# cxjyxxme/deep-online-video-stabilization

Measured on NVIDIA B200. Metric: warp_fwd_bwd_mpix_per_s, higher is better.
Workload: dtype f32

## Files before the change

### deep-online-video-stabilization_b200/csrc/mgw_warp_tma.cu

```cuda
#include "mgw_tile.cuh"

#ifdef MGW_PROBE
__device__ unsigned long long g_probe[16];
extern "C" __attribute__((visibility("default"))) int mgw_debug_probe(unsigned long long* out, int reset)
{
    cudaDeviceSynchronize();
    cudaMemcpyFromSymbol(out, g_probe, sizeof(g_probe));
    if (reset) { unsigned long long z[16] = {}; cudaMemcpyToSymbol(g_probe, z, sizeof(z)); }
    return 0;
}
#define PROBE(i) do { if (threadIdx.x == MGW_PROBE_TID) { const long long t_ = clock64(); atomicAdd(&g_probe[i], (unsigned long long)(t_ - tprev)); tprev = t_; } } while (0)
#else
#define PROBE(i) do {} while (0)
#endif
#ifndef MGW_PROBE_TID
#define MGW_PROBE_TID 32
#endif

namespace mgw {

constexpr int kMaxWarps = 16;

template <int C, int TW, int K, int NT>
struct Geo {
    static constexpr int kGroups = NT / TW;
    static constexpr int TH = kGroups * K;
    static constexpr int kXalign = (C % 4 == 0) ? 1 : ((C % 2 == 0) ? 2 : 4);
    static constexpr int kWantF = (((TW * 13 + 9) / 10 + 4 + (kXalign - 1)) * C + 31) / 32 * 32;
    static constexpr int kRowF = kWantF < 256 ? kWantF : 256;
    static constexpr int SBW = kRowF / C;
    static constexpr int SBH = (TH * 13 + 9) / 10 + 4;
    static constexpr int kBoxF = SBH * kRowF;
    static constexpr int kOutF = (TH * TW * C + 31) / 32 * 32;
    static_assert(SBW >= TW + 4, "source box too narrow for this tile width / channel count");
};

struct TileInfo {
    int bx0, by0;
    int interior;
    float wmax[kMaxWarps];
};

struct Tile {
    int n, r0, c0, vr0, vc0, cell, part;
};

__device__ __forceinline__ Tile this_tile(const TileCfg& cfg)
{
    Tile t;
    const int ty = blockIdx.y, tx = blockIdx.x;
    t.n = blockIdx.z;
    t.r0 = cfg.rows.start[ty]; t.vr0 = cfg.rows.vstart[ty];
    t.c0 = cfg.cols.start[tx]; t.vc0 = cfg.cols.vstart[tx];
    t.cell = (t.n * cfg.gh + cfg.rows.cell[ty]) * cfg.gw + cfg.cols.cell[tx];
    t.part = cfg.rows.part[ty] * cfg.parts_x + cfg.cols.part[tx];
    return t;
}

template <int C, int TW, int K, int NT>
__device__ __forceinline__ void source_box(const TileCfg& cfg, const Tile& tl, const float (&Hc)[9], float stepx, float stepy,
                                           int& bx0, int& by0, int& interior, int* complete = nullptr)
{
    using G = Geo<C, TW, K, NT>;
    const int k4 = threadIdx.x & 3;
    const int rr = tl.r0 + ((k4 & 2) ? G::TH - 1 : 0), cc = tl.c0 + ((k4 & 1) ? TW - 1 : 0);
    const Proj q = project(Hc, lin_at(cc, stepx), lin_at(rr, stepy));
    const float x = (q.xn + 1.0f) * (float)cfg.W * 0.5f, y = (q.yn + 1.0f) * (float)cfg.H * 0.5f;
    bool ok = (fabsf(x) < 1.0e8f) && (fabsf(y) < 1.0e8f);
    int sgn = (q.zs > 0.0f) ? 1 : -1;
    float xmin = x, xmax = x, ymin = y, ymax = y;
#pragma unroll
    for (int o = 1; o < 4; o <<= 1) {
        xmin = fminf(xmin, __shfl_xor_sync(0xffffffffu, xmin, o));
        xmax = fmaxf(xmax, __shfl_xor_sync(0xffffffffu, xmax, o));
        ymin = fminf(ymin, __shfl_xor_sync(0xffffffffu, ymin, o));
        ymax = fmaxf(ymax, __shfl_xor_sync(0xffffffffu, ymax, o));
        sgn += __shfl_xor_sync(0xffffffffu, sgn, o);
        ok = ok && (__shfl_xor_sync(0xffffffffu, (int)ok, o) != 0);
    }
    ok = ok && (sgn == 4 || sgn == -4);
    bx0 = 0; by0 = 0; interior = 0;
    if (complete) *complete = 0;
    if (ok) {
        const int ux0 = (int)floorf(xmin) - 1, ux1 = (int)floorf(xmax) + 2;
        const int uy0 = (int)floorf(ymin) - 1, uy1 = (int)floorf(ymax) + 2;
        const int ix0 = clipi(ux0, 0, cfg.W - 1), ix1 = clipi(ux1, 0, cfg.W - 1);
        const int iy0 = clipi(uy0, 0, cfg.H - 1), iy1 = clipi(uy1, 0, cfg.H - 1);
        const int needw = ix1 - ix0 + 1, needh = iy1 - iy0 + 1;
        bx0 = needw <= G::SBW ? ix0 : ix0 + (needw - G::SBW) / 2;
        by0 = needh <= G::SBH ? iy0 : iy0 + (needh - G::SBH) / 2;
        bx0 -= bx0 % G::kXalign;
        interior = (ux0 >= 0 && ux1 <= cfg.W - 1 && uy0 >= 0 && uy1 <= cfg.H - 1 &&
                    ux1 - bx0 < G::SBW && uy1 - by0 < G::SBH) ? 1 : 0;
        if (complete) *complete = (ix0 >= bx0 && ix1 - bx0 < G::SBW && iy0 >= by0 && iy1 - by0 < G::SBH) ? 1 : 0;
    }
}

struct FastTaps { int x0, y0; float ax, bx, ay, by; };
__device__ __forceinline__ FastTaps make_taps_interior(float xn, float yn, int IH, int IW)
{
    const float x = __fmul_rn(__fmul_rn(__fadd_rn(xn, 1.0f), (float)IW), 0.5f);
    const float y = __fmul_rn(__fmul_rn(__fadd_rn(yn, 1.0f), (float)IH), 0.5f);
    const float fx = floorf(x), fy = floorf(y);
    FastTaps t;
    t.x0 = __float2int_rz(fx); t.y0 = __float2int_rz(fy);
    t.ax = __fsub_rn(__fadd_rn(fx, 1.0f), x); t.bx = __fsub_rn(x, fx);
    t.ay = __fsub_rn(__fadd_rn(fy, 1.0f), y); t.by = __fsub_rn(y, fy);
    return t;
}

__device__ __forceinline__ float blend4(float ax, float bx, float ay, float by, float Ia, float Ib, float Ic, float Id)
{
    const float wa = __fmul_rn(ax, ay), wb = __fmul_rn(ax, by), wc = __fmul_rn(bx, ay), wd = __fmul_rn(bx, by);
    float s = __fmul_rn(wa, Ia);
    s = __fadd_rn(s, __fmul_rn(wb, Ib));
    s = __fadd_rn(s, __fmul_rn(wc, Ic));
    s = __fadd_rn(s, __fmul_rn(wd, Id));
    return s;
}

#ifndef MGW_FWD_MINB
#define MGW_FWD_MINB (NT == 256 ? (LOSS ? 3 : 4) : 2)
#endif
template <int C, int TW, int K, int NT, bool LOSS>
__global__ void __launch_bounds__(NT, MGW_FWD_MINB)
warp_fwd_tma_kernel(const __grid_constant__ CUtensorMap mapU, const __grid_constant__ CUtensorMap mapOut,
                    const float* __restrict__ U, const float* __restrict__ Hs, const __grid_constant__ TileCfg cfg,
                    float* __restrict__ out, float* __restrict__ img, float* __restrict__ black,
                    const float* __restrict__ y_tgt, float* __restrict__ sums)
{
    using G = Geo<C, TW, K, NT>;
    extern __shared__ __align__(1024) unsigned char smem_raw[];
    float* s_src = reinterpret_cast<float*>(smem_raw);
    float* s_out = s_src + G::kBoxF;
    uint64_t* bar = reinterpret_cast<uint64_t*>(s_out + G::kOutF);
    TileInfo* ti = reinterpret_cast<TileInfo*>(bar + 2);

    const int tid = threadIdx.x;
    if (tid == 0) {
        tma::mbar_init(bar, 1);
        tma::fence_barrier_init();
    }
    const Tile tl = this_tile(cfg);
    float Hc[9];
#pragma unroll
    for (int k = 0; k < 9; ++k) Hc[k] = __ldg(Hs + (size_t)tl.cell * 9 + k);
    const float stepx = cfg.stepx, stepy = cfg.stepy;
    __syncthreads();
    if (tid < 32 && out) {
        int bx0, by0, interior;
        source_box<C, TW, K, NT>(cfg, tl, Hc, stepx, stepy, bx0, by0, interior);
        if (tid == 0) {
            ti->bx0 = bx0; ti->by0 = by0; ti->interior = interior;
            tma::mbar_expect_tx(bar, (uint32_t)(G::kBoxF * sizeof(float)));
            tma::load_3d(s_src, &mapU, bar, bx0 * C, by0, tl.n);
        }
    }

    const int tx = tid % TW, g = tid / TW;
    const float xt = lin_at(tl.c0 + tx, stepx);
    const float hx0 = __fmul_rn(Hc[0], xt), hx3 = __fmul_rn(Hc[3], xt), hx6 = __fmul_rn(Hc[6], xt);
    float xn[K], yn[K];
    float yv[LOSS ? K : 1][C], nbv[LOSS ? K : 1];
    {
        size_t p = ((size_t)tl.n * cfg.H + tl.r0 + g * K) * cfg.W + tl.c0 + tx;
#pragma unroll
        for (int k = 0; k < K; ++k, p += cfg.W) {
            if (LOSS) {
#pragma unroll
                for (int ch = 0; ch < C; ++ch) yv[k][ch] = __ldg(y_tgt + p * C + ch);
            }
            const float yt = lin_at(tl.r0 + g * K + k, stepy);
            const float xs = __fadd_rn(__fmaf_rn(Hc[1], yt, hx0), Hc[2]);
            const float ys = __fadd_rn(__fmaf_rn(Hc[4], yt, hx3), Hc[5]);
            float zs = __fadd_rn(__fmaf_rn(Hc[7], yt, hx6), Hc[8]);
            zs = __fadd_rn(zs, (zs >= 0.0f) ? 1e-8f : -1e-8f);
            div2_rn(xs, ys, zs, xn[k], yn[k]);
            const float bk = black_of(xn[k], yn[k]);
            if (img) reinterpret_cast<float2*>(img)[p] = make_float2(xn[k], yn[k]);
            if (black) black[p] = bk;
            if (LOSS) nbv[k] = (tl.r0 + g * K + k >= tl.vr0 && tl.c0 + tx >= tl.vc0) ? 1.0f - bk : -1.0f;
        }
    }
    if (!out) return;
    float se = 0.0f, sm = 0.0f;
    tma::mbar_wait(bar, 0);
    const int bx0 = ti->bx0, by0 = ti->by0;
    if (ti->interior) {
#pragma unroll
        for (int k = 0; k < K; ++k) {
            const FastTaps t = make_taps_interior(xn[k], yn[k], cfg.H, cfg.W);
            const float* pa = s_src + ((t.y0 - by0) * G::kRowF + (t.x0 - bx0) * C);
            float* o = s_out + ((g * K + k) * TW + tx) * C;
#pragma unroll
            for (int ch = 0; ch < C; ++ch) {
                const float v = blend4(t.ax, t.bx, t.ay, t.by, pa[ch], pa[G::kRowF + ch], pa[C + ch], pa[G::kRowF + C + ch]);
                o[ch] = v;
                if (LOSS && nbv[k] >= 0.0f) { const float e = (v - yv[k][ch]) * nbv[k]; se = fmaf(e, e, se); }
            }
            if (LOSS && nbv[k] >= 0.0f) sm += nbv[k];
        }
    } else {
        const float* Un = U + (size_t)tl.n * cfg.H * cfg.W * C;
#pragma unroll
        for (int k = 0; k < K; ++k) {
            const Taps t = make_taps(xn[k], yn[k], cfg.H, cfg.W);
            const int sx0 = t.x0 - bx0, sx1 = t.x1 - bx0, sy0 = t.y0 - by0, sy1 = t.y1 - by0;
            float* o = s_out + ((g * K + k) * TW + tx) * C;
            if (sx0 >= 0 && sx1 < G::SBW && sy0 >= 0 && sy1 < G::SBH) {
                const float* pa = s_src + sy0 * G::kRowF + sx0 * C;
                const float* pb = s_src + sy1 * G::kRowF + sx0 * C;
                const float* pc = s_src + sy0 * G::kRowF + sx1 * C;
                const float* pd = s_src + sy1 * G::kRowF + sx1 * C;
#pragma unroll
                for (int ch = 0; ch < C; ++ch) o[ch] = blend(t, pa[ch], pb[ch], pc[ch], pd[ch]);
            } else {
                const float* pa = Un + ((size_t)t.y0 * cfg.W + t.x0) * C;
                const float* pb = Un + ((size_t)t.y1 * cfg.W + t.x0) * C;
                const float* pc = Un + ((size_t)t.y0 * cfg.W + t.x1) * C;
                const float* pd = Un + ((size_t)t.y1 * cfg.W + t.x1) * C;
#pragma unroll
                for (int ch = 0; ch < C; ++ch) o[ch] = blend(t, __ldg(pa + ch), __ldg(pb + ch), __ldg(pc + ch), __ldg(pd + ch));
            }
            if (LOSS && nbv[k] >= 0.0f) {
#pragma unroll
                for (int ch = 0; ch < C; ++ch) { const float e = (o[ch] - yv[k][ch]) * nbv[k]; se = fmaf(e, e, se); }
                sm += nbv[k];
            }
        }
    }
    if (LOSS) {
        se = warp_sum(se); sm = warp_sum(sm);
        float* s_loss = reinterpret_cast<float*>(ti + 1);
        if ((tid & 31) == 0) { s_loss[(tid >> 5) * 2] = se; s_loss[(tid >> 5) * 2 + 1] = sm; }
    }
    tma::fence_proxy_async();
    __syncthreads();
    if (tid == 0) {
        tma::store_3d(&mapOut, s_out, tl.c0 * C, tl.r0, tl.n);
        tma::commit_group();
        if (LOSS) {
            const float* s_loss = reinterpret_cast<const float*>(ti + 1);
            float a = 0.0f, b = 0.0f;
#pragma unroll
            for (int w = 0; w < NT / 32; ++w) { a += s_loss[2 * w]; b += s_loss[2 * w + 1]; }
            atomicAdd(sums + 2 * tl.n, a);
            atomicAdd(sums + 2 * tl.n + 1, b);
        }
        tma::wait_group_read0();
    }
}

constexpr float kMagic = 12582912.0f;
constexpr int kMagicBits = 0x4B400000;
__device__ __forceinline__ int fixed_of(float w, float gs) { return __float_as_int(__fmaf_rn(w, gs, kMagic)) - kMagicBits; }
__device__ __forceinline__ float float_of_fixed(int v) { return (float)v; }
constexpr int bit_width(int v) { return v > 0 ? 1 + bit_width(v >> 1) : 0; }

__device__ __forceinline__ void accumulate_dh(float (&dh)[8], float gxn, float gyn, float xn, float yn, float zs, float xt, float yt)
{
    const float rz = __frcp_rn(zs);
    const float dxs = gxn * rz, dys = gyn * rz;
    const float dzs = -(gxn * xn + gyn * yn) * rz;
    dh[0] = fmaf(dxs, xt, dh[0]); dh[1] = fmaf(dxs, yt, dh[1]); dh[2] += dxs;
    dh[3] = fmaf(dys, xt, dh[3]); dh[4] = fmaf(dys, yt, dh[4]); dh[5] += dys;
    dh[6] = fmaf(dzs, xt, dh[6]); dh[7] = fmaf(dzs, yt, dh[7]);
}

__device__ __forceinline__ void accumulate_dh_r(float (&dh)[8], float gxn, float gyn, float xn, float yn, float rz, float xt, float yt)
{
    const float dxs = gxn * rz, dys = gyn * rz;
    const float dzs = -(gxn * xn + gyn * yn) * rz;
    dh[0] = fmaf(dxs, xt, dh[0]); dh[1] = fmaf(dxs, yt, dh[1]); dh[2] += dxs;
    dh[3] = fmaf(dys, xt, dh[3]); dh[4] = fmaf(dys, yt, dh[4]); dh[5] += dys;
    dh[6] = fmaf(dzs, xt, dh[6]); dh[7] = fmaf(dzs, yt, dh[7]);
}

struct LossBwd {
    const float* out;
    const float* y;
    const float* black;
    const float* sums;
    float kscale;
    const float* kscale_dev;
};

#ifndef MGW_BWD_MINB
#define MGW_BWD_MINB (NT == 256 ? (K <= 3 ? 4 : 3) : 2)
#endif
#ifndef MGW_BWD_NODU_MINB
#define MGW_BWD_NODU_MINB (NT == 256 ? 4 : 2)
#endif
template <int C, int TW, int K, int NT, bool LOSS, bool DU>
__global__ void __launch_bounds__(NT, DU ? MGW_BWD_MINB : MGW_BWD_NODU_MINB)
warp_bwd_tma_kernel(const __grid_constant__ CUtensorMap mapU, const __grid_constant__ CUtensorMap mapG,
                    const __grid_constant__ CUtensorMap mapGI, const float* __restrict__ U, const float* __restrict__ Hs, const float* __restrict__ d_out,
                    const float* __restrict__ d_img, const __grid_constant__ TileCfg cfg, float* __restrict__ dU,
                    float* __restrict__ parts, const LossBwd loss)
{
    using G = Geo<C, TW, K, NT>;
    extern __shared__ __align__(1024) unsigned char smem_raw[];
    float* s_src = reinterpret_cast<float*>(smem_raw);
    float* s_red = s_src + G::kBoxF;
    uint64_t* bar = reinterpret_cast<uint64_t*>(s_red + 128);
    TileInfo* ti = reinterpret_cast<TileInfo*>(bar + 2);
    int* s_acc = reinterpret_cast<int*>(s_red + 256);

    constexpr bool STAGE = DU && !LOSS && (G::kBoxF >= G::TH * TW * (C + 2));
    constexpr int kStageOut = G::TH * TW * C;
    const int tid = threadIdx.x, lane = tid & 31, warp = tid >> 5;
#ifdef MGW_PROBE
    long long tprev = clock64();
    if (tid == MGW_PROBE_TID) atomicAdd(&g_probe[15], 1ull);
#endif
    if (tid == 0) {
        tma::mbar_init(bar, 1);
        if (STAGE) tma::mbar_init(bar + 1, 1);
        tma::fence_barrier_init();
    }
    griddep_launch_dependents();
    PROBE(11);
    const Tile tl = this_tile(cfg);
    PROBE(12);
    if (STAGE && tid == 0) {
        float* sg = reinterpret_cast<float*>(s_acc);
        tma::mbar_expect_tx(bar + 1, (uint32_t)((kStageOut + (d_img ? G::TH * TW * 2 : 0)) * sizeof(float)));
        tma::load_3d(sg, &mapG, bar + 1, tl.c0 * C, tl.r0, tl.n);
        if (d_img) tma::load_3d(sg + kStageOut, &mapGI, bar + 1, tl.c0 * 2, tl.r0, tl.n);
    }
    float Hc[9];
#pragma unroll
    for (int k = 0; k < 9; ++k) Hc[k] = __ldg(Hs + (size_t)tl.cell * 9 + k);
    const float stepx = cfg.stepx, stepy = cfg.stepy;
    const int tx = tid % TW, g = tid / TW;
    const int col = tl.c0 + tx;

    if (tid < 32) {
        int bx0, by0, interior, complete;
        source_box<C, TW, K, NT>(cfg, tl, Hc, stepx, stepy, bx0, by0, interior, &complete);
        if (tid == 0) {
            ti->bx0 = bx0; ti->by0 = by0; ti->interior = complete;
            tma::mbar_expect_tx(bar, (uint32_t)(G::kBoxF * sizeof(float)));
            tma::load_3d(s_src, &mapU, bar, bx0 * C, by0, tl.n);
        }
    }
    PROBE(13);
    float gout[K][C], gimg[K][2];
    if (STAGE) {
        __syncthreads();
        tma::mbar_wait(bar + 1, 0);
        const float* sg = reinterpret_cast<const float*>(s_acc) + (g * K * TW + tx) * C;
        const float2* si = reinterpret_cast<const float2*>(reinterpret_cast<const float*>(s_acc) + kStageOut) + g * K * TW + tx;
#pragma unroll
        for (int k = 0; k < K; ++k) {
#pragma unroll
            for (int ch = 0; ch < C; ++ch) gout[k][ch] = sg[k * TW * C + ch];
            if (d_img) {
                const float2 di = si[k * TW];
                gimg[k][0] = di.x; gimg[k][1] = di.y;
            } else {
                gimg[k][0] = 0.0f; gimg[k][1] = 0.0f;
            }
        }
    } else {
        size_t p = ((size_t)tl.n * cfg.H + tl.r0 + g * K) * cfg.W + col;
        const float kn = LOSS ? (loss.kscale_dev ? loss.kscale * __ldg(loss.kscale_dev) : loss.kscale) / (__ldg(loss.sums + 2 * tl.n + 1) + 1e-8f) : 0.0f;
#pragma unroll
        for (int k = 0; k < K; ++k, p += cfg.W) {
            if (LOSS) {
                const float nb = 1.0f - __ldg(loss.black + p);
                const float kk = kn * nb * nb;
#pragma unroll
                for (int ch = 0; ch < C; ++ch) {
                    gout[k][ch] = kk * (__ldg(loss.out + p * C + ch) - __ldg(loss.y + p * C + ch));
                    if (d_out) gout[k][ch] += __ldg(d_out + p * C + ch);
                }
            } else {
#pragma unroll
                for (int ch = 0; ch < C; ++ch) gout[k][ch] = __ldg(d_out + p * C + ch);
            }
            if (d_img) {
                const float2 di = __ldg(reinterpret_cast<const float2*>(d_img) + p);
                gimg[k][0] = di.x; gimg[k][1] = di.y;
            } else {
                gimg[k][0] = 0.0f; gimg[k][1] = 0.0f;
            }
        }
    }
    PROBE(0);
    if (DU) {
        unsigned m = 0u;
#pragma unroll
        for (int k = 0; k < K; ++k)
#pragma unroll
            for (int ch = 0; ch < C; ++ch) m = max(m, (unsigned)__float_as_int(gout[k][ch]) & 0x7fffffffu);
        m = __reduce_max_sync(0xffffffffu, m);
        if (lane == 0) ti->wmax[warp] = __int_as_float((int)m);
    }
    if (DU) {
        if (STAGE) __syncthreads();
        int4* a4 = reinterpret_cast<int4*>(s_acc);
#pragma unroll
        for (int i = 0; i < (G::kBoxF / 4 + NT - 1) / NT; ++i)
            if (i * NT + tid < G::kBoxF / 4) a4[i * NT + tid] = make_int4(0, 0, 0, 0);
    }
    PROBE(1);
    __syncthreads();
    PROBE(2);
    const int bx0 = ti->bx0, by0 = ti->by0;
    int fixed = 0;
    float scale = 0.0f, inv_scale = 0.0f;
    if (DU) {
        unsigned mb = 0u;
#pragma unroll
        for (int w = 0; w < NT / 32; ++w) mb = max(mb, (unsigned)__float_as_int(ti->wmax[w]));
        const float mm = __int_as_float((int)mb);
        const int e = (int)(mb >> 23) - 127;
        constexpr int kTerms = G::TH * TW;
        constexpr int kBits = 31 - bit_width(kTerms);
        static_assert(kBits <= 22 && ((long long)kTerms << kBits) < (1LL << 31), "fixed-point headroom");
        fixed = (mm > 0.0f) && (e > -100) && (e < 100);
        scale = __int_as_float((kBits - 1 - e + 127) << 23);
        inv_scale = __int_as_float((e - (kBits - 1) + 127) << 23);
    }

    const float xt = lin_at(col, stepx);
    const float hx0 = __fmul_rn(Hc[0], xt), hx3 = __fmul_rn(Hc[3], xt), hx6 = __fmul_rn(Hc[6], xt);
    float dh[8];
#pragma unroll
    for (int k = 0; k < 8; ++k) dh[k] = 0.0f;
    const float halfW = 0.5f * (float)cfg.W, halfH = 0.5f * (float)cfg.H;

    PROBE(3);
    tma::mbar_wait(bar, 0);
    PROBE(4);
    if (ti->interior && (fixed || !DU)) {
#pragma unroll
        for (int k = 0; k < K; ++k) {
            const int row = tl.r0 + g * K + k;
            if (row >= tl.vr0 && col >= tl.vc0) {
                const float yt = lin_at(row, stepy);
                const float xs = __fadd_rn(__fmaf_rn(Hc[1], yt, hx0), Hc[2]);
                const float ys = __fadd_rn(__fmaf_rn(Hc[4], yt, hx3), Hc[5]);
                float zs = __fadd_rn(__fmaf_rn(Hc[7], yt, hx6), Hc[8]);
                zs = __fadd_rn(zs, (zs >= 0.0f) ? 1e-8f : -1e-8f);
                float xn, yn;
                const float rz = div2_rn(xs, ys, zs, xn, yn);
                const FastTaps t = make_taps_interior(xn, yn, cfg.H, cfg.W);
                float gx = 0.0f, gy = 0.0f;
                if ((unsigned)t.x0 < (unsigned)(cfg.W - 1) && (unsigned)t.y0 < (unsigned)(cfg.H - 1)) {
                    const int ia = ((t.y0 - by0) * G::kRowF + (t.x0 - bx0) * C);
                    const float* pa = s_src + ia;
                    int* qa = s_acc + ia;
                    const float wa = t.ax * t.ay, wb = t.ax * t.by, wc = t.bx * t.ay, wd = t.bx * t.by;
                    float sa = 0.0f, sb = 0.0f, sc = 0.0f, sd = 0.0f;
#pragma unroll
                    for (int ch = 0; ch < C; ++ch) {
                        const float gch = gout[k][ch];
                        sa = fmaf(gch, pa[ch], sa); sb = fmaf(gch, pa[G::kRowF + ch], sb);
                        sc = fmaf(gch, pa[C + ch], sc); sd = fmaf(gch, pa[G::kRowF + C + ch], sd);
                        if (DU) {
                            const float gs = gch * scale;
                            atomicAdd(qa + ch, fixed_of(wa, gs));
                            atomicAdd(qa + G::kRowF + ch, fixed_of(wb, gs));
                            atomicAdd(qa + C + ch, fixed_of(wc, gs));
                            atomicAdd(qa + G::kRowF + C + ch, fixed_of(wd, gs));
                        }
                    }
                    gx = fmaf(sc - sa, t.ay, (sd - sb) * t.by); gy = fmaf(sb - sa, t.ax, (sd - sc) * t.bx);
                }
                accumulate_dh_r(dh, fmaf(gx, halfW, gimg[k][0]), fmaf(gy, halfH, gimg[k][1]), xn, yn, rz, xt, yt);
            }
        }
    } else {
        if (DU) griddep_wait();
        const float* Un = U + (size_t)tl.n * cfg.H * cfg.W * C;
        float* dUn = DU ? dU + (size_t)tl.n * cfg.H * cfg.W * C : nullptr;
#pragma unroll
        for (int k = 0; k < K; ++k) {
            const int row = tl.r0 + g * K + k;
            if (row >= tl.vr0 && col >= tl.vc0) {
                const float yt = lin_at(row, stepy);
                const float xs = __fadd_rn(__fmaf_rn(Hc[1], yt, hx0), Hc[2]);
                const float ys = __fadd_rn(__fmaf_rn(Hc[4], yt, hx3), Hc[5]);
                float zs = __fadd_rn(__fmaf_rn(Hc[7], yt, hx6), Hc[8]);
                zs = __fadd_rn(zs, (zs >= 0.0f) ? 1e-8f : -1e-8f);
                const float xn = __fdiv_rn(xs, zs), yn = __fdiv_rn(ys, zs);
                const Taps t = make_taps(xn, yn, cfg.H, cfg.W);
                const int sx0 = t.x0 - bx0, sx1 = t.x1 - bx0, sy0 = t.y0 - by0, sy1 = t.y1 - by0;
                const bool inbox = sx0 >= 0 && sx1 < G::SBW && sy0 >= 0 && sy1 < G::SBH;
                const float wa = t.ax * t.ay, wb = t.ax * t.by, wc = t.bx * t.ay, wd = t.bx * t.by;
                float gx = 0.0f, gy = 0.0f;
                const bool scatter = DU && taps_scatter(t);
                const size_t ga = ((size_t)t.y0 * cfg.W + t.x0) * C, gb = ((size_t)t.y1 * cfg.W + t.x0) * C;
                const size_t gc = ((size_t)t.y0 * cfg.W + t.x1) * C, gd = ((size_t)t.y1 * cfg.W + t.x1) * C;
                const int ia = sy0 * G::kRowF + sx0 * C, ib = sy1 * G::kRowF + sx0 * C;
                const int ic = sy0 * G::kRowF + sx1 * C, id = sy1 * G::kRowF + sx1 * C;
#pragma unroll
                for (int ch = 0; ch < C; ++ch) {
                    const float gch = gout[k][ch];
                    float Ia, Ib, Ic, Id;
                    if (inbox) { Ia = s_src[ia + ch]; Ib = s_src[ib + ch]; Ic = s_src[ic + ch]; Id = s_src[id + ch]; }
                    else { Ia = __ldg(Un + ga + ch); Ib = __ldg(Un + gb + ch); Ic = __ldg(Un + gc + ch); Id = __ldg(Un + gd + ch); }
                    gx = fmaf(gch, fmaf(Ic - Ia, t.ay, (Id - Ib) * t.by), gx);
                    gy = fmaf(gch, fmaf(Ib - Ia, t.ax, (Id - Ic) * t.bx), gy);
                    if (scatter) {
                        if (inbox && fixed) {
                            const float gs = gch * scale;
                            atomicAdd(s_acc + ia + ch, fixed_of(wa, gs));
                            atomicAdd(s_acc + ib + ch, fixed_of(wb, gs));
                            atomicAdd(s_acc + ic + ch, fixed_of(wc, gs));
                            atomicAdd(s_acc + id + ch, fixed_of(wd, gs));
                        } else {
                            atomicAdd(dUn + ga + ch, wa * gch);
                            atomicAdd(dUn + gb + ch, wb * gch);
                            atomicAdd(dUn + gc + ch, wc * gch);
                            atomicAdd(dUn + gd + ch, wd * gch);
                        }
                    }
                }
                accumulate_dh(dh, fmaf(gx, halfW, gimg[k][0]), fmaf(gy, halfH, gimg[k][1]), xn, yn, zs, xt, yt);
            }
        }
    }
    PROBE(5);
    {
        float v4[4], v2[2], v1;
        const bool hi16 = lane & 16, hi8 = lane & 8, hi4 = lane & 4;
#pragma unroll
        for (int i = 0; i < 4; ++i) {
            const float send = hi16 ? dh[i] : dh[i + 4], keep = hi16 ? dh[i + 4] : dh[i];
            v4[i] = keep + __shfl_xor_sync(0xffffffffu, send, 16);
        }
#pragma unroll
        for (int i = 0; i < 2; ++i) {
            const float send = hi8 ? v4[i] : v4[i + 2], keep = hi8 ? v4[i + 2] : v4[i];
            v2[i] = keep + __shfl_xor_sync(0xffffffffu, send, 8);
        }
        {
            const float send = hi4 ? v2[0] : v2[1], keep = hi4 ? v2[1] : v2[0];
            v1 = keep + __shfl_xor_sync(0xffffffffu, send, 4);
        }
        v1 += __shfl_xor_sync(0xffffffffu, v1, 2);
        v1 += __shfl_xor_sync(0xffffffffu, v1, 1);
        if ((lane & 3) == 0) s_red[warp * 8 + ((lane >> 4) & 1) * 4 + ((lane >> 3) & 1) * 2 + ((lane >> 2) & 1)] = v1;
    }
    PROBE(6);
    __syncthreads();
    PROBE(7);
    if (tid < 8) {
        float v = 0.0f;
#pragma unroll
        for (int w = 0; w < NT / 32; ++w) v += s_red[w * 8 + tid];
        parts[((size_t)tl.cell * (cfg.parts_y * cfg.parts_x) + tl.part) * 8 + tid] = v;
    }
    if (fixed) {
        griddep_wait();
        const int4* a4 = reinterpret_cast<const int4*>(s_acc);
        constexpr int kQ = G::kRowF / 4;
        const int rows = min(G::SBH, cfg.H - by0);
        const int nq = min(G::kRowF, (cfg.W - bx0) * C) / 4;
        float* base = dU + (((size_t)tl.n * cfg.H + by0) * cfg.W + bx0) * C;
        const int pitch = cfg.W * C;
#pragma unroll
        for (int i = 0; i < (G::kBoxF / 4 + NT - 1) / NT; ++i) {
            const int j = i * NT + tid;
            const int row = j / kQ, q = j % kQ;
            if (row < rows && q < nq) {
                const int4 v = a4[j];
                if ((v.x | v.y | v.z | v.w) != 0)
                    tma::red_add_v4(base + row * pitch + q * 4, float_of_fixed(v.x) * inv_scale, float_of_fixed(v.y) * inv_scale,
                                    float_of_fixed(v.z) * inv_scale, float_of_fixed(v.w) * inv_scale);
            }
        }
        PROBE(8);
    }
}

struct Plan {
    TileCfg cfg;
    int TW, K, NT, TH, nty, ntx;
};

constexpr int kNumVariants = 6;
static const int kVariants[kNumVariants][3] = {{64, 6, 256}, {64, 3, 512}, {64, 3, 256}, {32, 3, 256}, {32, 2, 256}, {32, 1, 256}};

static bool plan(const WarpShape& s, Plan* out)
{
    if (s.OH != s.H || s.OW != s.W) return false;
    if (s.C != 1 && s.C != 3 && s.C != 4) return false;
    if (s.H > 65535 || s.W > 65535 || s.gh > 255 || s.gw > 255 || s.N > 65535) return false;
    const int cell_h = s.H / s.gh, cell_w = s.W / s.gw;
    if (s.W % 4 != 0 || cell_w % 4 != 0) return false;
    double best_eff = 0;
    int best = -1;
    for (int v = 0; v < kNumVariants; ++v) {
        const int tw = kVariants[v][0], k = kVariants[v][1], th = (kVariants[v][2] / tw) * k;
        if (tw > cell_w || th > cell_h) continue;
        if (s.C == 4 && tw == 64) continue;
        const double ey = (double)cell_h / (((cell_h + th - 1) / th) * th), ex = (double)cell_w / (((cell_w + tw - 1) / tw) * tw);
        const double eff = ey * ex * (tw == 64 ? 1.0 : 0.93) * (th >= 12 ? 1.0 : 0.9);
        if (eff > best_eff) { best_eff = eff; best = v; }
    }
    if (const char* force = getenv("MGW_TILE")) {
        int tw = 0, k = 0, nt = 256;
        if (sscanf(force, "%dx%dx%d", &tw, &k, &nt) >= 2)
            for (int v = 0; v < kNumVariants; ++v)
                if (kVariants[v][0] == tw && kVariants[v][1] == k && kVariants[v][2] == nt && tw <= cell_w && (nt / tw) * k <= cell_h &&
                    !(s.C == 4 && tw == 64)) best = v;
    }
    if (best < 0) return false;
    Plan p;
    p.TW = kVariants[best][0]; p.K = kVariants[best][1]; p.NT = kVariants[best][2]; p.TH = (p.NT / p.TW) * p.K;
    TileCfg& c = p.cfg;
    c.N = s.N; c.H = s.H; c.W = s.W; c.gh = s.gh; c.gw = s.gw;
    tile_steps(&c);
    p.nty = fill_axis(&c.rows, s.gh, cell_h, s.H, p.TH, &c.parts_y);
    p.ntx = fill_axis(&c.cols, s.gw, cell_w, s.W, p.TW, &c.parts_x);
    if (p.nty < 0 || p.ntx < 0 || c.parts_y > 255 || c.parts_x > 255) return false;
    *out = p;
    return true;
}

bool tma_fwd_supported(const WarpShape& s) { Plan p; return plan(s, &p); }
bool tma_bwd_supported(const WarpShape& s) { Plan p; return plan(s, &p); }

size_t tma_bwd_workspace_bytes(const WarpShape& s)
{
    Plan p;
    if (!plan(s, &p)) return 0;
    return (size_t)s.N * s.gh * s.gw * p.cfg.parts_y * p.cfg.parts_x * 8 * sizeof(float);
}

template <int C, int TW, int K, int NT>
static int launch_fwd_v(const float* U, const float* Hs, const Plan& p, float* out, float* black, float* img, const float* y_tgt,
                        float* sums, cudaStream_t st)
{
    using G = Geo<C, TW, K, NT>;
    const TileCfg& c = p.cfg;
    CUtensorMap mU, mOut;
    TRY_RC(make_map(&mU, U, c.W * C, c.H, c.N, G::kRowF, G::SBH));
    TRY_RC(make_map(&mOut, out ? out : U, c.W * C, c.H, c.N, TW * C, G::TH));
    const size_t smem = (size_t)(G::kBoxF + G::kOutF) * 4 + 16 + sizeof(TileInfo) + 2 * kMaxWarps * 4 + 64;
    if (y_tgt) {
        static bool attr_l[64] = {};
        TRY_RC(allow_smem(warp_fwd_tma_kernel<C, TW, K, NT, true>, attr_l, "warp_fwd_tma(loss)"));
        warp_fwd_tma_kernel<C, TW, K, NT, true><<<dim3(p.ntx, p.nty, c.N), NT, smem, st>>>(mU, mOut, U, Hs, c, out, img, black, y_tgt, sums);
        return check_launch("warp_fwd_tma(loss)");
    }
    static bool attr[64] = {};
    TRY_RC(allow_smem(warp_fwd_tma_kernel<C, TW, K, NT, false>, attr, "warp_fwd_tma"));
    warp_fwd_tma_kernel<C, TW, K, NT, false><<<dim3(p.ntx, p.nty, c.N), NT, smem, st>>>(mU, mOut, U, Hs, c, out, img, black, nullptr, nullptr);
    return check_launch("warp_fwd_tma");
}

template <int C, int TW, int K, int NT>
static int launch_bwd_v(const float* U, const float* Hs, const float* d_out, const float* d_img, const Plan& p, float* dU,
                        float* parts, const LossBwd* loss, cudaStream_t st, bool behind_own_fill)
{
    using G = Geo<C, TW, K, NT>;
    const TileCfg& c = p.cfg;
    CUtensorMap mU;
    TRY_RC(make_map(&mU, U, c.W * C, c.H, c.N, G::kRowF, G::SBH));
    CUtensorMap mG = mU, mGI = mU;
    if (dU && !loss) {
        TRY_RC(make_map(&mG, d_out, c.W * C, c.H, c.N, TW * C, G::TH));
        if (d_img) TRY_RC(make_map(&mGI, d_img, c.W * 2, c.H, c.N, TW * 2, G::TH));
    }
    size_t smem = (size_t)(G::kBoxF + 256 + (dU ? G::kBoxF : 0)) * 4 + 64;
    if (const char* e = getenv("MGW_BWD_PAD_SMEM")) smem += (size_t)atoi(e);
    const dim3 grid(p.ntx, p.nty, c.N);
    if (loss && dU) {
        static bool attr[64] = {};
        TRY_RC(allow_smem(warp_bwd_tma_kernel<C, TW, K, NT, true, true>, attr, "warp_bwd_tma(loss)"));
        warp_bwd_tma_kernel<C, TW, K, NT, true, true><<<grid, NT, smem, st>>>(mU, mG, mGI, U, Hs, d_out, d_img, c, dU, parts, *loss);
    } else if (loss) {
        static bool attr[64] = {};
        TRY_RC(allow_smem(warp_bwd_tma_kernel<C, TW, K, NT, true, false>, attr, "warp_bwd_tma(loss, no dU)"));
        warp_bwd_tma_kernel<C, TW, K, NT, true, false><<<grid, NT, smem, st>>>(mU, mG, mGI, U, Hs, d_out, d_img, c, nullptr, parts, *loss);
    } else if (dU) {
        static bool attr[64] = {};
        TRY_RC(allow_smem(warp_bwd_tma_kernel<C, TW, K, NT, false, true>, attr, "warp_bwd_tma"));
        const cudaError_t e = launch_ex(warp_bwd_tma_kernel<C, TW, K, NT, false, true>, grid, dim3(NT), smem, st, behind_own_fill && pdl_enabled(),
                                        mU, mG, mGI, U, Hs, d_out, d_img, c, dU, parts, LossBwd{});
        if (e != cudaSuccess) { count_launches(1); return set_error(MGW_ERR_CUDA, "warp_bwd_tma: %s", cudaGetErrorString(e)); }
    } else {
        static bool attr[64] = {};
        TRY_RC(allow_smem(warp_bwd_tma_kernel<C, TW, K, NT, false, false>, attr, "warp_bwd_tma(no dU)"));
        warp_bwd_tma_kernel<C, TW, K, NT, false, false><<<grid, NT, smem, st>>>(mU, mG, mGI, U, Hs, d_out, d_img, c, nullptr, parts, LossBwd{});
    }
    return check_launch("warp_bwd_tma");
}

template <int C>
static int launch_fwd_c(const Plan& p, const float* U, const float* Hs, float* out, float* black, float* img, const float* y_tgt,
                        float* sums, cudaStream_t st)
{
    if (p.NT == 256 && p.TW == 32 && p.K == 3) return launch_fwd_v<C, 32, 3, 256>(U, Hs, p, out, black, img, y_tgt, sums, st);
    if (p.NT == 256 && p.TW == 32 && p.K == 2) return launch_fwd_v<C, 32, 2, 256>(U, Hs, p, out, black, img, y_tgt, sums, st);
    if (p.NT == 256 && p.TW == 32 && p.K == 1) return launch_fwd_v<C, 32, 1, 256>(U, Hs, p, out, black, img, y_tgt, sums, st);
    if constexpr (C != 4) {
        if (p.NT == 256 && p.TW == 64 && p.K == 6) return launch_fwd_v<C, 64, 6, 256>(U, Hs, p, out, black, img, y_tgt, sums, st);
        if (p.NT == 512 && p.TW == 64 && p.K == 3) return launch_fwd_v<C, 64, 3, 512>(U, Hs, p, out, black, img, y_tgt, sums, st);
        if (p.NT == 256 && p.TW == 64 && p.K == 3) return launch_fwd_v<C, 64, 3, 256>(U, Hs, p, out, black, img, y_tgt, sums, st);
    }
    return set_error(MGW_ERR_UNSUPPORTED, "warp_fwd_tma: no tile variant");
}

template <int C>
static int launch_bwd_c(const Plan& p, const float* U, const float* Hs, const float* d_out, const float* d_img, float* dU,
                        float* parts, const LossBwd* loss, cudaStream_t st, bool behind_own_fill)
{
    if (p.NT == 256 && p.TW == 32 && p.K == 3) return launch_bwd_v<C, 32, 3, 256>(U, Hs, d_out, d_img, p, dU, parts, loss, st, behind_own_fill);
    if (p.NT == 256 && p.TW == 32 && p.K == 2) return launch_bwd_v<C, 32, 2, 256>(U, Hs, d_out, d_img, p, dU, parts, loss, st, behind_own_fill);
    if (p.NT == 256 && p.TW == 32 && p.K == 1) return launch_bwd_v<C, 32, 1, 256>(U, Hs, d_out, d_img, p, dU, parts, loss, st, behind_own_fill);
    if constexpr (C != 4) {
        if (p.NT == 256 && p.TW == 64 && p.K == 6) return launch_bwd_v<C, 64, 6, 256>(U, Hs, d_out, d_img, p, dU, parts, loss, st, behind_own_fill);
        if (p.NT == 512 && p.TW == 64 && p.K == 3) return launch_bwd_v<C, 64, 3, 512>(U, Hs, d_out, d_img, p, dU, parts, loss, st, behind_own_fill);
        if (p.NT == 256 && p.TW == 64 && p.K == 3) return launch_bwd_v<C, 64, 3, 256>(U, Hs, d_out, d_img, p, dU, parts, loss, st, behind_own_fill);
    }
    return set_error(MGW_ERR_UNSUPPORTED, "warp_bwd_tma: no tile variant");
}

int launch_warp_fwd_tma(const float* U, const float* Hs, const WarpShape& s, float* out, float* black, float* img,
                        const float* y_tgt, float* sums, cudaStream_t st)
{
    Plan p;
    if (!plan(s, &p)) return set_error(MGW_ERR_UNSUPPORTED, "warp_fwd_tma: unsupported shape");
    if (s.C == 1) return launch_fwd_c<1>(p, U, Hs, out, black, img, y_tgt, sums, st);
    if (s.C == 3) return launch_fwd_c<3>(p, U, Hs, out, black, img, y_tgt, sums, st);
    return launch_fwd_c<4>(p, U, Hs, out, black, img, y_tgt, sums, st);
}

int launch_warp_bwd_tma(const float* U, const float* Hs, const float* d_out, const float* d_img, const WarpShape& s, float* dU,
                        float* parts, int* nparts, const FusedImgLoss* fl, cudaStream_t st, bool behind_own_fill)
{
    LossBwd lb{};
    const LossBwd* loss = nullptr;
    if (fl) { lb.out = fl->out; lb.y = fl->y; lb.black = fl->black; lb.sums = fl->sums; lb.kscale = fl->kscale; lb.kscale_dev = fl->kscale_dev; loss = &lb; }
    Plan p;
    if (!plan(s, &p)) return set_error(MGW_ERR_UNSUPPORTED, "warp_bwd_tma: unsupported shape");
    *nparts = p.cfg.parts_y * p.cfg.parts_x;
    const int cell_h = s.H / s.gh, cell_w = s.W / s.gw;
    const bool all_slots_written = (s.H % s.gh == 0) && (s.W % s.gw == 0) && (p.nty == s.gh * ((cell_h + p.TH - 1) / p.TH)) &&
                                   (p.ntx == s.gw * ((cell_w + p.TW - 1) / p.TW));
    if (!all_slots_written && cudaMemsetAsync(parts, 0, tma_bwd_workspace_bytes(s), st) != cudaSuccess)
        return set_error(MGW_ERR_CUDA, "memset parts: %s", cudaGetErrorString(cudaGetLastError()));
    if (!all_slots_written) behind_own_fill = false;
    if (s.C == 1) return launch_bwd_c<1>(p, U, Hs, d_out, d_img, dU, parts, loss, st, behind_own_fill);
    if (s.C == 3) return launch_bwd_c<3>(p, U, Hs, d_out, d_img, dU, parts, loss, st, behind_own_fill);
    return launch_bwd_c<4>(p, U, Hs, d_out, d_img, dU, parts, loss, st, behind_own_fill);
}

}
```

Measured before the change: 43420.

## Split backward into gather then scatter phase reusing source smem as accumulator

Result: slower. 42900 (median of 6 runs) (-1.2%).

```diff
diff --git a/deep-online-video-stabilization_b200/csrc/mgw_warp_tma.cu b/deep-online-video-stabilization_b200/csrc/mgw_warp_tma.cu
--- a/deep-online-video-stabilization_b200/csrc/mgw_warp_tma.cu
+++ b/deep-online-video-stabilization_b200/csrc/mgw_warp_tma.cu
@@ -97,16 +97,19 @@
 }
 
 struct FastTaps { int x0, y0; float ax, bx, ay, by; };
-__device__ __forceinline__ FastTaps make_taps_interior(float xn, float yn, int IH, int IW)
-{
-    const float x = __fmul_rn(__fmul_rn(__fadd_rn(xn, 1.0f), (float)IW), 0.5f);
-    const float y = __fmul_rn(__fmul_rn(__fadd_rn(yn, 1.0f), (float)IH), 0.5f);
+__device__ __forceinline__ float pixel_of(float vn, int size) { return __fmul_rn(__fmul_rn(__fadd_rn(vn, 1.0f), (float)size), 0.5f); }
+__device__ __forceinline__ FastTaps taps_at(float x, float y)
+{
     const float fx = floorf(x), fy = floorf(y);
     FastTaps t;
     t.x0 = __float2int_rz(fx); t.y0 = __float2int_rz(fy);
     t.ax = __fsub_rn(__fadd_rn(fx, 1.0f), x); t.bx = __fsub_rn(x, fx);
     t.ay = __fsub_rn(__fadd_rn(fy, 1.0f), y); t.by = __fsub_rn(y, fy);
     return t;
+}
+__device__ __forceinline__ FastTaps make_taps_interior(float xn, float yn, int IH, int IW)
+{
+    return taps_at(pixel_of(xn, IW), pixel_of(yn, IH));
 }
 
 __device__ __forceinline__ float blend4(float ax, float bx, float ay, float by, float Ia, float Ib, float Ic, float Id)
@@ -286,28 +289,27 @@
 };
 
 #ifndef MGW_BWD_MINB
-#define MGW_BWD_MINB (NT == 256 ? (K <= 3 ? 4 : 3) : 2)
-#endif
-#ifndef MGW_BWD_NODU_MINB
-#define MGW_BWD_NODU_MINB (NT == 256 ? 4 : 2)
+#define MGW_BWD_MINB (NT == 256 ? 4 : 2)
 #endif
 template <int C, int TW, int K, int NT, bool LOSS, bool DU>
-__global__ void __launch_bounds__(NT, DU ? MGW_BWD_MINB : MGW_BWD_NODU_MINB)
+__global__ void __launch_bounds__(NT, MGW_BWD_MINB)
 warp_bwd_tma_kernel(const __grid_constant__ CUtensorMap mapU, const __grid_constant__ CUtensorMap mapG,
-                    const __grid_constant__ CUtensorMap mapGI, const float* __restrict__ U, const float* __restrict__ Hs, const float* __restrict__ d_out,
+                    const float* __restrict__ U, const float* __restrict__ Hs, const float* __restrict__ d_out,
                     const float* __restrict__ d_img, const __grid_constant__ TileCfg cfg, float* __restrict__ dU,
                     float* __restrict__ parts, const LossBwd loss)
 {
     using G = Geo<C, TW, K, NT>;
     extern __shared__ __align__(1024) unsigned char smem_raw[];
     float* s_src = reinterpret_cast<float*>(smem_raw);
+    int* s_acc = reinterpret_cast<int*>(s_src);
     float* s_red = s_src + G::kBoxF;
     uint64_t* bar = reinterpret_cast<uint64_t*>(s_red + 128);
     TileInfo* ti = reinterpret_cast<TileInfo*>(bar + 2);
-    int* s_acc = reinterpret_cast<int*>(s_red + 256);
-
-    constexpr bool STAGE = DU && !LOSS && (G::kBoxF >= G::TH * TW * (C + 2));
+    float* s_g = s_red + 256;
+
+    constexpr bool STAGE = DU && !LOSS;
     constexpr int kStageOut = G::TH * TW * C;
+    static_assert(kStageOut % 4 == 0, "the staged d_out tile is read in 16-byte groups");
     const int tid = threadIdx.x, lane = tid & 31, warp = tid >> 5;
 #ifdef MGW_PROBE
     long long tprev = clock64();
@@ -323,10 +325,8 @@
     const Tile tl = this_tile(cfg);
     PROBE(12);
     if (STAGE && tid == 0) {
-        float* sg = reinterpret_cast<float*>(s_acc);
-        tma::mbar_expect_tx(bar + 1, (uint32_t)((kStageOut + (d_img ? G::TH * TW * 2 : 0)) * sizeof(float)));
-        tma::load_3d(sg, &mapG, bar + 1, tl.c0 * C, tl.r0, tl.n);
-        if (d_img) tma::load_3d(sg + kStageOut, &mapGI, bar + 1, tl.c0 * 2, tl.r0, tl.n);
+        tma::mbar_expect_tx(bar + 1, (uint32_t)(kStageOut * sizeof(float)));
+        tma::load_3d(s_g, &mapG, bar + 1, tl.c0 * C, tl.r0, tl.n);
     }
     float Hc[9];
 #pragma unroll
@@ -345,24 +345,9 @@
         }
     }
     PROBE(13);
-    float gout[K][C], gimg[K][2];
-    if (STAGE) {
-        __syncthreads();
-        tma::mbar_wait(bar + 1, 0);
-        const float* sg = reinterpret_cast<const float*>(s_acc) + (g * K * TW + tx) * C;
-        const float2* si = reinterpret_cast<const float2*>(reinterpret_cast<const float*>(s_acc) + kStageOut) + g * K * TW + tx;
-#pragma unroll
-        for (int k = 0; k < K; ++k) {
-#pragma unroll
-            for (int ch = 0; ch < C; ++ch) gout[k][ch] = sg[k * TW * C + ch];
-            if (d_img) {
-                const float2 di = si[k * TW];
-                gimg[k][0] = di.x; gimg[k][1] = di.y;
-            } else {
-                gimg[k][0] = 0.0f; gimg[k][1] = 0.0f;
-            }
-        }
-    } else {
+    float gout[DU ? 1 : K][C], gimg[K][2];
+    const int own = (g * K * TW + tx) * C;
+    {
         size_t p = ((size_t)tl.n * cfg.H + tl.r0 + g * K) * cfg.W + col;
         const float kn = LOSS ? (loss.kscale_dev ? loss.kscale * __ldg(loss.kscale_dev) : loss.kscale) / (__ldg(loss.sums + 2 * tl.n + 1) + 1e-8f) : 0.0f;
 #pragma unroll
@@ -372,12 +357,14 @@
                 const float kk = kn * nb * nb;
 #pragma unroll
                 for (int ch = 0; ch < C; ++ch) {
-                    gout[k][ch] = kk * (__ldg(loss.out + p * C + ch) - __ldg(loss.y + p * C + ch));
-                    if (d_out) gout[k][ch] += __ldg(d_out + p * C + ch);
+                    float v = kk * (__ldg(loss.out + p * C + ch) - __ldg(loss.y + p * C + ch));
+                    if (d_out) v += __ldg(d_out + p * C + ch);
+                    if (DU) s_g[own + k * TW * C + ch] = v;
+                    else gout[DU ? 0 : k][ch] = v;
                 }
-            } else {
-#pragma unroll
-                for (int ch = 0; ch < C; ++ch) gout[k][ch] = __ldg(d_out + p * C + ch);
+            } else if (!DU) {
+#pragma unroll
+                for (int ch = 0; ch < C; ++ch) gout[DU ? 0 : k][ch] = __ldg(d_out + p * C + ch);
             }
             if (d_img) {
                 const float2 di = __ldg(reinterpret_cast<const float2*>(d_img) + p);
@@ -389,20 +376,27 @@
     }
     PROBE(0);
     if (DU) {
+        if (STAGE) {
+            __syncthreads();
+            tma::mbar_wait(bar + 1, 0);
+        }
         unsigned m = 0u;
-#pragma unroll
-        for (int k = 0; k < K; ++k)
-#pragma unroll
-            for (int ch = 0; ch < C; ++ch) m = max(m, (unsigned)__float_as_int(gout[k][ch]) & 0x7fffffffu);
+        if (STAGE) {
+            const uint4* g4 = reinterpret_cast<const uint4*>(s_g);
+#pragma unroll
+            for (int i = 0; i < (kStageOut / 4 + NT - 1) / NT; ++i)
+                if (i * NT + tid < kStageOut / 4) {
+                    const uint4 v = g4[i * NT + tid];
+                    m = max(max(m, max(v.x & 0x7fffffffu, v.y & 0x7fffffffu)), max(v.z & 0x7fffffffu, v.w & 0x7fffffffu));
+                }
+        } else {
+#pragma unroll
+            for (int k = 0; k < K; ++k)
+#pragma unroll
+                for (int ch = 0; ch < C; ++ch) m = max(m, (unsigned)__float_as_int(s_g[own + k * TW * C + ch]) & 0x7fffffffu);
+        }
         m = __reduce_max_sync(0xffffffffu, m);
         if (lane == 0) ti->wmax[warp] = __int_as_float((int)m);
-    }
-    if (DU) {
-        if (STAGE) __syncthreads();
-        int4* a4 = reinterpret_cast<int4*>(s_acc);
-#pragma unroll
-        for (int i = 0; i < (G::kBoxF / 4 + NT - 1) / NT; ++i)
-            if (i * NT + tid < G::kBoxF / 4) a4[i * NT + tid] = make_int4(0, 0, 0, 0);
     }
     PROBE(1);
     __syncthreads();
@@ -430,11 +424,14 @@
 #pragma unroll
     for (int k = 0; k < 8; ++k) dh[k] = 0.0f;
     const float halfW = 0.5f * (float)cfg.W, halfH = 0.5f * (float)cfg.H;
+    const float* sg = s_g + own;
+    float px[DU ? K : 1], py[DU ? K : 1];
 
     PROBE(3);
     tma::mbar_wait(bar, 0);
     PROBE(4);
-    if (ti->interior && (fixed || !DU)) {
+    const bool fast = ti->interior && (fixed || !DU);
+    if (fast) {
 #pragma unroll
         for (int k = 0; k < K; ++k) {
             const int row = tl.r0 + g * K + k;
@@ -446,26 +443,18 @@
                 zs = __fadd_rn(zs, (zs >= 0.0f) ? 1e-8f : -1e-8f);
                 float xn, yn;
                 const float rz = div2_rn(xs, ys, zs, xn, yn);
-                const FastTaps t = make_taps_interior(xn, yn, cfg.H, cfg.W);
+                const float x = pixel_of(xn, cfg.W), y = pixel_of(yn, cfg.H);
+                px[DU ? k : 0] = x; py[DU ? k : 0] = y;
+                const FastTaps t = taps_at(x, y);
                 float gx = 0.0f, gy = 0.0f;
                 if ((unsigned)t.x0 < (unsigned)(cfg.W - 1) && (unsigned)t.y0 < (unsigned)(cfg.H - 1)) {
-                    const int ia = ((t.y0 - by0) * G::kRowF + (t.x0 - bx0) * C);
-                    const float* pa = s_src + ia;
-                    int* qa = s_acc + ia;
-                    const float wa = t.ax * t.ay, wb = t.ax * t.by, wc = t.bx * t.ay, wd = t.bx * t.by;
+                    const float* pa = s_src + ((t.y0 - by0) * G::kRowF + (t.x0 - bx0) * C);
                     float sa = 0.0f, sb = 0.0f, sc = 0.0f, sd = 0.0f;
 #pragma unroll
                     for (int ch = 0; ch < C; ++ch) {
-                        const float gch = gout[k][ch];
+                        const float gch = DU ? sg[k * TW * C + ch] : gout[DU ? 0 : k][ch];
                         sa = fmaf(gch, pa[ch], sa); sb = fmaf(gch, pa[G::kRowF + ch], sb);
                         sc = fmaf(gch, pa[C + ch], sc); sd = fmaf(gch, pa[G::kRowF + C + ch], sd);
-                        if (DU) {
-                            const float gs = gch * scale;
-                            atomicAdd(qa + ch, fixed_of(wa, gs));
-                            atomicAdd(qa + G::kRowF + ch, fixed_of(wb, gs));
-                            atomicAdd(qa + C + ch, fixed_of(wc, gs));
-                            atomicAdd(qa + G::kRowF + C + ch, fixed_of(wd, gs));
-                        }
                     }
                     gx = fmaf(sc - sa, t.ay, (sd - sb) * t.by); gy = fmaf(sb - sa, t.ax, (sd - sc) * t.bx);
                 }
@@ -473,9 +462,7 @@
             }
         }
     } else {
-        if (DU) griddep_wait();
         const float* Un = U + (size_t)tl.n * cfg.H * cfg.W * C;
-        float* dUn = DU ? dU + (size_t)tl.n * cfg.H * cfg.W * C : nullptr;
 #pragma unroll
         for (int k = 0; k < K; ++k) {
             const int row = tl.r0 + g * K + k;
@@ -486,38 +473,23 @@
                 float zs = __fadd_rn(__fmaf_rn(Hc[7], yt, hx6), Hc[8]);
                 zs = __fadd_rn(zs, (zs >= 0.0f) ? 1e-8f : -1e-8f);
                 const float xn = __fdiv_rn(xs, zs), yn = __fdiv_rn(ys, zs);
+                px[DU ? k : 0] = xn; py[DU ? k : 0] = yn;
                 const Taps t = make_taps(xn, yn, cfg.H, cfg.W);
                 const int sx0 = t.x0 - bx0, sx1 = t.x1 - bx0, sy0 = t.y0 - by0, sy1 = t.y1 - by0;
                 const bool inbox = sx0 >= 0 && sx1 < G::SBW && sy0 >= 0 && sy1 < G::SBH;
-                const float wa = t.ax * t.ay, wb = t.ax * t.by, wc = t.bx * t.ay, wd = t.bx * t.by;
                 float gx = 0.0f, gy = 0.0f;
-                const bool scatter = DU && taps_scatter(t);
                 const size_t ga = ((size_t)t.y0 * cfg.W + t.x0) * C, gb = ((size_t)t.y1 * cfg.W + t.x0) * C;
                 const size_t gc = ((size_t)t.y0 * cfg.W + t.x1) * C, gd = ((size_t)t.y1 * cfg.W + t.x1) * C;
                 const int ia = sy0 * G::kRowF + sx0 * C, ib = sy1 * G::kRowF + sx0 * C;
                 const int ic = sy0 * G::kRowF + sx1 * C, id = sy1 * G::kRowF + sx1 * C;
 #pragma unroll
                 for (int ch = 0; ch < C; ++ch) {
-                    const float gch = gout[k][ch];
+                    const float gch = DU ? sg[k * TW * C + ch] : gout[DU ? 0 : k][ch];
                     float Ia, Ib, Ic, Id;
                     if (inbox) { Ia = s_src[ia + ch]; Ib = s_src[ib + ch]; Ic = s_src[ic + ch]; Id = s_src[id + ch]; }
                     else { Ia = __ldg(Un + ga + ch); Ib = __ldg(Un + gb + ch); Ic = __ldg(Un + gc + ch); Id = __ldg(Un + gd + ch); }
                     gx = fmaf(gch, fmaf(Ic - Ia, t.ay, (Id - Ib) * t.by), gx);
                     gy = fmaf(gch, fmaf(Ib - Ia, t.ax, (Id - Ic) * t.bx), gy);
-                    if (scatter) {
-                        if (inbox && fixed) {
-                            const float gs = gch * scale;
-                            atomicAdd(s_acc + ia + ch, fixed_of(wa, gs));
-                            atomicAdd(s_acc + ib + ch, fixed_of(wb, gs));
-                            atomicAdd(s_acc + ic + ch, fixed_of(wc, gs));
-                            atomicAdd(s_acc + id + ch, fixed_of(wd, gs));
-                        } else {
-                            atomicAdd(dUn + ga + ch, wa * gch);
-                            atomicAdd(dUn + gb + ch, wb * gch);
-                            atomicAdd(dUn + gc + ch, wc * gch);
-                            atomicAdd(dUn + gd + ch, wd * gch);
-                        }
-                    }
                 }
                 accumulate_dh(dh, fmaf(gx, halfW, gimg[k][0]), fmaf(gy, halfH, gimg[k][1]), xn, yn, zs, xt, yt);
             }
@@ -546,8 +518,76 @@
         if ((lane & 3) == 0) s_red[warp * 8 + ((lane >> 4) & 1) * 4 + ((lane >> 3) & 1) * 2 + ((lane >> 2) & 1)] = v1;
     }
     PROBE(6);
+    if (DU) {
+        __syncthreads();
+        int4* a4 = reinterpret_cast<int4*>(s_acc);
+#pragma unroll
+        for (int i = 0; i < (G::kBoxF / 4 + NT - 1) / NT; ++i)
+            if (i * NT + tid < G::kBoxF / 4) a4[i * NT + tid] = make_int4(0, 0, 0, 0);
+        __syncthreads();
+        PROBE(7);
+        if (fast) {
+#pragma unroll
+            for (int k = 0; k < K; ++k) {
+                const int row = tl.r0 + g * K + k;
+                if (row >= tl.vr0 && col >= tl.vc0) {
+                    const FastTaps t = taps_at(px[k], py[k]);
+                    if ((unsigned)t.x0 < (unsigned)(cfg.W - 1) && (unsigned)t.y0 < (unsigned)(cfg.H - 1)) {
+                        int* qa = s_acc + ((t.y0 - by0) * G::kRowF + (t.x0 - bx0) * C);
+                        const float wa = t.ax * t.ay, wb = t.ax * t.by, wc = t.bx * t.ay, wd = t.bx * t.by;
+#pragma unroll
+                        for (int ch = 0; ch < C; ++ch) {
+                            const float gs = sg[k * TW * C + ch] * scale;
+                            atomicAdd(qa + ch, fixed_of(wa, gs));
+                            atomicAdd(qa + G::kRowF + ch, fixed_of(wb, gs));
+                            atomicAdd(qa + C + ch, fixed_of(wc, gs));
+                            atomicAdd(qa + G::kRowF + C + ch, fixed_of(wd, gs));
+                        }
+                    }
+                }
+            }
+        } else {
+            griddep_wait();
+            float* dUn = dU + (size_t)tl.n * cfg.H * cfg.W * C;
+#pragma unroll
+            for (int k = 0; k < K; ++k) {
+                const int row = tl.r0 + g * K + k;
+                if (row >= tl.vr0 && col >= tl.vc0) {
+                    const Taps t = make_taps(px[k], py[k], cfg.H, cfg.W);
+                    if (taps_scatter(t)) {
+                        const int sx0 = t.x0 - bx0, sx1 = t.x1 - bx0, sy0 = t.y0 - by0, sy1 = t.y1 - by0;
+                        const float wa = t.ax * t.ay, wb = t.ax * t.by, wc = t.bx * t.ay, wd = t.bx * t.by;
+                        if (fixed && sx0 >= 0 && sx1 < G::SBW && sy0 >= 0 && sy1 < G::SBH) {
+                            const int ia = sy0 * G::kRowF + sx0 * C, ib = sy1 * G::kRowF + sx0 * C;
+                            const int ic = sy0 * G::kRowF + sx1 * C, id = sy1 * G::kRowF + sx1 * C;
+#pragma unroll
+                            for (int ch = 0; ch < C; ++ch) {
+                                const float gs = sg[k * TW * C + ch] * scale;
+                                atomicAdd(s_acc + ia + ch, fixed_of(wa, gs));
+                                atomicAdd(s_acc + ib + ch, fixed_of(wb, gs));
+                                atomicAdd(s_acc + ic + ch, fixed_of(wc, gs));
+                                atomicAdd(s_acc + id + ch, fixed_of(wd, gs));
+                            }
+                        } else {
+                            const size_t ga = ((size_t)t.y0 * cfg.W + t.x0) * C, gb = ((size_t)t.y1 * cfg.W + t.x0) * C;
+                            const size_t gc = ((size_t)t.y0 * cfg.W + t.x1) * C, gd = ((size_t)t.y1 * cfg.W + t.x1) * C;
+#pragma unroll
+                            for (int ch = 0; ch < C; ++ch) {
+                                const float gch = sg[k * TW * C + ch];
+                                atomicAdd(dUn + ga + ch, wa * gch);
+                                atomicAdd(dUn + gb + ch, wb * gch);
+                                atomicAdd(dUn + gc + ch, wc * gch);
+                                atomicAdd(dUn + gd + ch, wd * gch);
+                            }
+                        }
+                    }
+                }
+            }
+        }
+        PROBE(8);
+    }
     __syncthreads();
-    PROBE(7);
+    PROBE(9);
     if (tid < 8) {
         float v = 0.0f;
 #pragma unroll
@@ -573,7 +613,7 @@
                                     float_of_fixed(v.z) * inv_scale, float_of_fixed(v.w) * inv_scale);
             }
         }
-        PROBE(8);
+        PROBE(10);
     }
 }
 
@@ -662,32 +702,29 @@
     const TileCfg& c = p.cfg;
     CUtensorMap mU;
     TRY_RC(make_map(&mU, U, c.W * C, c.H, c.N, G::kRowF, G::SBH));
-    CUtensorMap mG = mU, mGI = mU;
-    if (dU && !loss) {
-        TRY_RC(make_map(&mG, d_out, c.W * C, c.H, c.N, TW * C, G::TH));
-        if (d_img) TRY_RC(make_map(&mGI, d_img, c.W * 2, c.H, c.N, TW * 2, G::TH));
-    }
-    size_t smem = (size_t)(G::kBoxF + 256 + (dU ? G::kBoxF : 0)) * 4 + 64;
+    CUtensorMap mG = mU;
+    if (dU && !loss) TRY_RC(make_map(&mG, d_out, c.W * C, c.H, c.N, TW * C, G::TH));
+    size_t smem = (size_t)(G::kBoxF + 256 + (dU ? G::TH * TW * C : 0)) * 4 + 64;
     if (const char* e = getenv("MGW_BWD_PAD_SMEM")) smem += (size_t)atoi(e);
     const dim3 grid(p.ntx, p.nty, c.N);
     if (loss && dU) {
         static bool attr[64] = {};
         TRY_RC(allow_smem(warp_bwd_tma_kernel<C, TW, K, NT, true, true>, attr, "warp_bwd_tma(loss)"));
-        warp_bwd_tma_kernel<C, TW, K, NT, true, true><<<grid, NT, smem, st>>>(mU, mG, mGI, U, Hs, d_out, d_img, c, dU, parts, *loss);
+        warp_bwd_tma_kernel<C, TW, K, NT, true, true><<<grid, NT, smem, st>>>(mU, mG, U, Hs, d_out, d_img, c, dU, parts, *loss);
     } else if (loss) {
         static bool attr[64] = {};
         TRY_RC(allow_smem(warp_bwd_tma_kernel<C, TW, K, NT, true, false>, attr, "warp_bwd_tma(loss, no dU)"));
-        warp_bwd_tma_kernel<C, TW, K, NT, true, false><<<grid, NT, smem, st>>>(mU, mG, mGI, U, Hs, d_out, d_img, c, nullptr, parts, *loss);
+        warp_bwd_tma_kernel<C, TW, K, NT, true, false><<<grid, NT, smem, st>>>(mU, mG, U, Hs, d_out, d_img, c, nullptr, parts, *loss);
     } else if (dU) {
         static bool attr[64] = {};
         TRY_RC(allow_smem(warp_bwd_tma_kernel<C, TW, K, NT, false, true>, attr, "warp_bwd_tma"));
         const cudaError_t e = launch_ex(warp_bwd_tma_kernel<C, TW, K, NT, false, true>, grid, dim3(NT), smem, st, behind_own_fill && pdl_enabled(),
-                                        mU, mG, mGI, U, Hs, d_out, d_img, c, dU, parts, LossBwd{});
+                                        mU, mG, U, Hs, d_out, d_img, c, dU, parts, LossBwd{});
         if (e != cudaSuccess) { count_launches(1); return set_error(MGW_ERR_CUDA, "warp_bwd_tma: %s", cudaGetErrorString(e)); }
     } else {
         static bool attr[64] = {};
         TRY_RC(allow_smem(warp_bwd_tma_kernel<C, TW, K, NT, false, false>, attr, "warp_bwd_tma(no dU)"));
-        warp_bwd_tma_kernel<C, TW, K, NT, false, false><<<grid, NT, smem, st>>>(mU, mG, mGI, U, Hs, d_out, d_img, c, nullptr, parts, LossBwd{});
+        warp_bwd_tma_kernel<C, TW, K, NT, false, false><<<grid, NT, smem, st>>>(mU, mG, U, Hs, d_out, d_img, c, nullptr, parts, LossBwd{});
     }
     return check_launch("warp_bwd_tma");
 }
```
